# ynalcakan/RGBX_Semantic_Segmentation

Measured on AMD Instinct MI355X. Metric: train images/sec CMX-B2 480x640 bs=2/GPU at 1/2/4/8 MI355X; % MFMA roofline, higher is better.
Workload: dtype bf16

## Files before the change

rgbx_semantic_segmentation_amd/csrc/gemm.hip:

```cpp
#include "gemm_kernels.h"
#include <string.h>
#include <stdlib.h>

using namespace gemmk;
namespace gp = gemmplan;
extern CMX_GEMM_FAST_INST(bf16)
extern CMX_GEMM_FAST_INST(f16)
extern CMX_GEMM_GENERIC_INST(float)
extern CMX_GEMM_GENERIC_INST(bf16)
extern CMX_GEMM_GENERIC_INST(f16)
static_assert(gp::FAST_BK == FBK && gp::GENERIC_BK == BK, "gemm_plan.h counts k-tiles of the kernels' depth");

namespace {
gp::GemmKnobs gemm_knobs() {
  gp::GemmKnobs k;
  k.tiles = cmx_knob("GEMM_TILES", k.tiles);
  k.smallk = cmx_knob("GEMM_SMALLK", k.smallk);
  k.t128 = cmx_knob("GEMM_T128", k.t128);
  k.splitkw = cmx_knob("GEMM_SPLITKW", k.splitkw);
  k.kw = cmx_knob("GEMM_KW", k.kw);
  k.mid = cmx_knob("GEMM_MID", k.mid);
  k.stream = cmx_knob("GEMM_STREAM", k.stream);
  k.stream_k = cmx_knob("GEMM_STREAM_K", k.stream_k);
  k.stream_bpc = cmx_knob("GEMM_STREAM_BPC", k.stream_bpc);
  k.grouped_kt = cmx_knob("GROUPED_KT", k.grouped_kt);
  return k;
}

int launch_gemm(const gp::GemmLaunch& L, const GemmArgs& a, int tA, int tB, int dtype, hipStream_t s) {
  bool ok = true;
  if (L.path == gp::PATH_STREAM) {
    if (dtype == 2) launch_stream<f16>(L, a, tB, s);
    else launch_stream<bf16>(L, a, tB, s);
  } else if (L.path == gp::PATH_TILE) ok = dtype == 2 ? launch_tile<f16>(L, a, tA, tB, s) : launch_tile<bf16>(L, a, tA, tB, s);
  else if (dtype == 1) ok = launch_generic<bf16>(L, a, tA, tB, s);
  else if (dtype == 2) ok = launch_generic<f16>(L, a, tA, tB, s);
  else ok = launch_generic<float>(L, a, tA, tB, s);
  CMX_REQUIRE(ok, CMX_ERR_LAUNCH, "gemm: no kernel for path %d, tile %d x %d, NS %d, KW %d", L.path, L.bm, L.bn, L.ns,
              L.kw);
  if (L.nsplit > 1) {
    if (dtype == 1) launch_reduce<bf16>(L, a, s);
    else if (dtype == 2) launch_reduce<f16>(L, a, s);
    else launch_reduce<float>(L, a, s);
  }
  return CMX_OK;
}

void set_plan(GemmArgs& a, const gp::GemmLaunch& L) {
  a.kt_per_split = L.kt_per_split; a.nsplit = L.nsplit; a.tiles_m = L.tiles_m; a.tiles_n = L.tiles_n;
}

struct RedRec {
  const float* src; float* dst; float* dst2;
  long sg, sb, dg, dg2;
  int ldd, ldd2, G, nblk, rows, cols, csplit, accumulate, zl, cpg, blk0, pad;
};

__global__ __launch_bounds__(256) void reduce_grouped_kernel(const RedRec* __restrict__ recs, int nrec) {
  __shared__ float red[256];
  const int b = blockIdx.x;
  int lo = 0, hi = nrec - 1;
  while (lo < hi) {
    const int mid = (lo + hi + 1) >> 1;
    if (recs[mid].blk0 <= b) lo = mid; else hi = mid - 1;
  }
  const RedRec& r = recs[lo];
  const int zl = r.zl, opb = 256 / zl;
  const int local = b - r.blk0;
  const int g = local / r.cpg, ch = local % r.cpg;
  const int o = threadIdx.x % opb, sl = threadIdx.x / opb;
  const long W = (long)r.rows * r.cols;
  const long w = (long)ch * opb + o;
  float s0 = 0.f, s1 = 0.f, s2 = 0.f, s3 = 0.f;
  if (w < W) {
    const float* p = r.src + (long)g * r.sg + w;
    const long sb = r.sb;
    int k = sl;
    for (; k + 3 * zl < r.nblk; k += 4 * zl) {
      s0 += p[(long)k * sb];
      s1 += p[(long)(k + zl) * sb];
      s2 += p[(long)(k + 2 * zl) * sb];
      s3 += p[(long)(k + 3 * zl) * sb];
    }
    for (; k < r.nblk; k += zl) s0 += p[(long)k * sb];
  }
  float v = (s0 + s1) + (s2 + s3);
// ... 114 lines not shown
              "bias-gradient / upsample / scatter", gh);
  a.gh = gh; a.sAh = p.sAh; a.sBh = p.sBh; a.sCh = p.sCh;
  if (nup) {
    CMX_REQUIRE(up->n <= 3 && G == 1 && !ones_col && N % 8 == 0 && (long)up->oH * up->oW > 0 &&
                M % (up->oH * up->oW) == 0, CMX_ERR_ARG, "gemm: upsample-add epilogue needs G = 1, N %% 8 == 0 and "
                "M a whole number of %d x %d grids", up->oH, up->oW);
    for (int q = 0; q < up->n; ++q) {
      CMX_REQUIRE(up->src[q] && ((uintptr_t)up->src[q] & 15) == 0 && up->h[q] > 0 && up->w[q] > 0, CMX_ERR_ARG,
                  "gemm: upsample-add source %d", q);
      a.up[q] = up->src[q]; a.uh[q] = up->h[q]; a.uw[q] = up->w[q];
    }
    a.nup = up->n; a.uoH = up->oH; a.uoW = up->oW;
  }
  if (p.scR > 0) {
    CMX_REQUIRE(G == 1 || p.sC > 0, CMX_ERR_ARG, "gemm: scatter");
    CMX_REQUIRE((!p.R || lnb) && out_mode == 0 && !ones_col && N == p.scR * p.scR * p.scC && M % (p.scHo * p.scWo) == 0,
                CMX_ERR_ARG, "gemm: patch scatter needs a plain store of N = R*R*C columns");
    a.scatter = 1; a.scH = p.scH; a.scW = p.scW; a.scC = p.scC; a.scR = p.scR; a.scHo = p.scHo; a.scWo = p.scWo;
  }
  set_plan(a, L);
  if (tail) {
    CMX_REQUIRE(fast && N <= 128 && N % 8 == 0 && splitk == 1 && !transA && !transB && out_mode == 0 && !ones_col &&
                    !a.nup && !a.scatter && gh == 1 && !p.mask && a.cvec && dtype != 0,
                CMX_ERR_ARG, "gemm_ln: the LayerNorm epilogue needs the 16-bit path without split-K, forward layouts, a "
                "plain aligned store and N <= 128, N %% 8 == 0 (G=%d M=%d N=%d K=%d)", G, M, N, K);
    CMX_REQUIRE(tail->gamma && tail->beta && tail->y && tail->mean && tail->rstd && ((uintptr_t)tail->y & 15) == 0 &&
                    tail->y != p.C, CMX_ERR_ARG, "gemm_ln: LayerNorm buffers");
    a.tail = 2; a.ln_gamma = tail->gamma; a.ln_beta = tail->beta; a.ln_sg = tail->sg; a.ln_y = tail->y;
    a.ln_mean = tail->mean; a.ln_rstd = tail->rstd; a.ln_eps = tail->eps;
  }
  if (lnb) {
    const bool al = ((uintptr_t)p.C & 15) == 0 && ((uintptr_t)lnb->x & 15) == 0 && ((uintptr_t)p.R & 15) == 0 &&
                    ((uintptr_t)lnb->dy2 & 15) == 0 && ((uintptr_t)lnb->dxs & 15) == 0;
    const bool rows_ok = a.scatter ? (p.scC == 64 || p.scC == 128) && p.scH == p.scHo * p.scR && p.scW == p.scWo * p.scR
                                   : N <= 128 && N % 8 == 0;
    CMX_REQUIRE(fast && splitk == 1 && !transA && transB && out_mode == 0 && !ones_col && !p.bias && p.act == 0 &&
                    !p.mask && !a.nup && gh == 1 && !p.A2 && a.cvec && al && rows_ok && dtype != 0 &&
                    !tail && lnb->x && lnb->gamma && lnb->mean && lnb->rstd && lnb->part && (!lnb->dxs || p.rscale),
                CMX_ERR_ARG, "gemm_ln_bwd: needs the 16-bit dgrad path (transB) without split-K, 16-B aligned rows, "
                "N <= 128 (N %% 8 == 0), no bias / activation (G=%d M=%d N=%d K=%d)", G, M, N, K);
    a.tail = 3; a.ln_gamma = lnb->gamma; a.ln_sg = lnb->sg; a.ln_mean = const_cast<float*>(lnb->mean); a.ln_rstd = const_cast<float*>(lnb->rstd);
    a.lnb_x = lnb->x; a.lnb_dy2 = lnb->dy2; a.lnb_dxs = lnb->dxs; a.lnb_part = lnb->part;
  }
  if (p.plan) {
    const int nblk = gp::multi_blocks(shape, L);
    if (!nblk) return 0;
    a.kt_per_split = (int)gp::cdiv(K, FBK);
    memset(p.plan, 0, sizeof(*p.plan));
    p.plan->a = a; p.plan->tA = transA; p.plan->tB = transB; p.plan->dtype = dtype;
    p.plan->nblk = nblk;
    p.plan->nk64 = a.kt_per_split;
    return nblk;
  }
  const int st = launch_gemm(L, a, transA, transB, dtype, s);
  return st != CMX_OK ? st : cmx_check_launch("gemm");
}
}

extern "C" {

int cmx_gemm(const void* A, const void* A2, const void* B, void* C, const float* bias, const void* R,
             const float* rscale, const void* mask, float* dbias, float* workspace, int G, int M, int N, int K, int K1,
             int64_t lda, int64_t lda2, int64_t ldb, int64_t ldc, int64_t sA, int64_t sA2, int64_t sB, int64_t sC,
             int64_t sbias, int64_t sdb, int rows_per_sample, int transA, int transB, int act, int out_mode,
             int ones_col, int splitk, int dtype, hipStream_t s) {
  GemmProblem p;
  p.A = A; p.A2 = A2; p.B = B; p.C = C; p.bias = bias; p.R = R; p.rscale = rscale; p.mask = mask; p.dbias = dbias;
  p.workspace = workspace; p.G = G; p.M = M; p.N = N; p.K = K; p.K1 = K1; p.lda = lda; p.lda2 = lda2; p.ldb = ldb;
  p.ldc = ldc; p.sA = sA; p.sA2 = sA2; p.sB = sB; p.sC = sC; p.sbias = sbias; p.sdb = sdb;
  p.rows_per_sample = rows_per_sample; p.transA = transA; p.transB = transB; p.act = act; p.out_mode = out_mode;
  p.ones_col = ones_col; p.splitk = splitk; p.dtype = dtype;
  return gemm_impl(p, s);
}

int cmx_gemm_ln(const void* A, const void* A2, const void* B, void* C, const float* bias, const void* R,
                const float* rscale, int G, int M, int N, int K, int K1, int64_t lda, int64_t lda2, int64_t ldb,
                int64_t ldc, int64_t sA, int64_t sA2, int64_t sB, int64_t sC, int64_t sbias, int rows_per_sample,
                int act, const float* ln_gamma, const float* ln_beta, int64_t ln_sg, float ln_eps, void* ln_y,
                float* ln_mean, float* ln_rstd, int dtype, hipStream_t s) {
  const LnTail t{ln_gamma, ln_beta, (long)ln_sg, ln_y, ln_mean, ln_rstd, ln_eps};
  GemmProblem p;
  p.A = A; p.A2 = A2; p.B = B; p.C = C; p.bias = bias; p.R = R; p.rscale = rscale;
  p.G = G; p.M = M; p.N = N; p.K = K; p.K1 = K1; p.lda = lda; p.lda2 = lda2; p.ldb = ldb; p.ldc = ldc;
  p.sA = sA; p.sA2 = sA2; p.sB = sB; p.sC = sC; p.sbias = sbias; p.rows_per_sample = rows_per_sample; p.act = act;
  p.splitk = 1; p.dtype = dtype; p.tail = &t;
  return gemm_impl(p, s);
}

int cmx_gemm_ln_bwd(const void* A, const void* B, void* dx, int G, int M, int N, int K, int64_t lda, int64_t ldb,
                    int64_t ldc, int64_t sA, int64_t sB, int64_t sC, const void* x, const float* gamma, int64_t sg,
                    const float* mean, const float* rstd, const void* dres, const void* dy2, const float* sscale,
                    int rows_per_sample, void* dxs, float* partials, int dtype, hipStream_t s) {
  const LnBwd l{x, gamma, (long)sg, mean, rstd, dy2, dxs, partials};
  GemmProblem p;
  p.A = A; p.B = B; p.C = dx; p.R = dres; p.rscale = sscale; p.G = G; p.M = M; p.N = N; p.K = K;
  p.lda = lda; p.ldb = ldb; p.ldc = ldc; p.sA = sA; p.sB = sB; p.sC = sC; p.rows_per_sample = rows_per_sample;
  p.transB = 1; p.splitk = 1; p.dtype = dtype; p.lnb = &l;
  return gemm_impl(p, s);
}


size_t cmx_gemm_ln_bwd_partials(int G, int M, int N) { return (size_t)G * ((M + 63) / 64) * 2 * N * sizeof(float); }

int cmx_conv_patch_dgrad_ln_bwd(const void* dy, const void* Wt, void* dx, int G, int NIg, int H, int Wd, int C, int R,
                                int Ho, int Wo, int N, int64_t sdy, int64_t sW, int64_t sdx, const void* x,
                                const float* gamma, int64_t sg, const float* mean, const float* rstd, const void* dres,
                                const void* dy2, const float* sscale, int rows_per_sample, void* dxs, float* partials,
// ... 153 lines not shown
                                   int splitk, int blk0) {
  const int M = NIg * Ho * Wo;
  CMX_REQUIRE(rec && G > 0 && N > 0 && C % 8 == 0 && N % 8 == 0 && M % 8 == 0 && tap >= 0 && tap < KH * KW,
              CMX_ERR_SHAPE, "gemm_group_pack_conv_wgrad: bad problem");
  CMX_REQUIRE(((uintptr_t)dy & 15) == 0 && ((uintptr_t)x & 15) == 0 && sdy % 8 == 0 && sx % 8 == 0, CMX_ERR_ARG,
              "gemm_group_pack_conv_wgrad: alignment");
  CMX_REQUIRE((long)NIg * H * Wd * C < (1L << 30) && (long)M * N < (1L << 30), CMX_ERR_SHAPE,
              "gemm_group_pack_conv_wgrad: too large for 31-bit offsets");
  const int ones = dbias ? 1 : 0;
  const int Nk = C + ones;
  const gp::GemmLaunch L = gp::plan_grouped(G, N, C, M, splitk, gemm_knobs());
  CMX_REQUIRE((splitk > 0 ? splitk : L.nsplit) == 1 || workspace, CMX_ERR_ARG,
              "gemm_group_pack_conv_wgrad: split-K needs a workspace");
  GroupRec r{};
  GemmArgs& a = r.a;
  a.A = dy; a.B = x; a.C = dW + (long)tap * C; a.dbias = dbias; a.ws = workspace;
  a.G = G; a.M = N; a.N = Nk; a.K = M; a.K1 = M; a.rows_per_sample = 1;
  a.out_mode = 1; a.ones_col = ones; a.vec = 1;
  a.lda = N; a.sA = sdy; a.ldb = 0; a.sB = sx; a.ldc = (long)KH * KW * C; a.sC = sdW; a.sdb = sdb;
  a.cvec = (((uintptr_t)a.C % 16) == 0) && (a.ldc * 4) % 16 == 0 && (sdW * 4) % 16 == 0;
  a.conv = 2; a.cH = H; a.cW = Wd; a.cC = C; a.cKW = KW; a.cst = stride; a.cpad = pad; a.cHo = Ho; a.cWo = Wo;
  a.ctap = tap;
  set_plan(a, L);
  r.bm = L.bm; r.bn = L.bn;
  r.blk0 = blk0;
  r.nblk = (int)L.grid_x;
  memcpy(rec, &r, sizeof(r));
  return r.nblk;
}

int cmx_conv_implicit_fwd(const void* x, const void* Wt, void* y, const float* bias, float* workspace, int G, int NIg,
                          int H, int Wd, int C, int KH, int KW, int stride, int pad, int Ho, int Wo, int N, int64_t sx,
                          int64_t sW, int64_t sy, int64_t sbias, int splitk, int dtype, hipStream_t s) {
  CMX_REQUIRE((dtype == 1 || dtype == 2) && C % 64 == 0 && N % 8 == 0 && G > 0 && NIg > 0, CMX_ERR_SHAPE,
              "conv_implicit_fwd: bf16 / fp16 with C %% 64 == 0 only (C=%d, N=%d)", C, N);
  CMX_REQUIRE(((uintptr_t)x & 15) == 0 && ((uintptr_t)Wt & 15) == 0 && ((uintptr_t)y & 15) == 0 && sx % 8 == 0 &&
              sW % 8 == 0 && sy % 8 == 0, CMX_ERR_ARG, "conv_implicit_fwd: alignment");
  const long M = (long)NIg * Ho * Wo, K = (long)KH * KW * C;
  CMX_REQUIRE((long)NIg * H * Wd * C < (1L << 30) && M * N < (1L << 31) && (long)N * K < (1L << 30), CMX_ERR_SHAPE,
              "conv_implicit_fwd: too large for 31-bit offsets");
  GemmArgs a{};
  a.A = x; a.B = Wt; a.C = y; a.bias = bias;
  a.G = G; a.M = (int)M; a.N = N; a.K = (int)K; a.K1 = (int)K; a.rows_per_sample = 1; a.vec = 1;
  a.lda = 0; a.sA = sx; a.ldb = K; a.sB = sW; a.ldc = N; a.sC = sy; a.sbias = sbias;
  a.cvec = (N * 2) % 16 == 0 && (sy * 2) % 16 == 0;
  a.conv = 1; a.cH = H; a.cW = Wd; a.cC = C; a.cKW = KW; a.cst = stride; a.cpad = pad; a.cHo = Ho; a.cWo = Wo;
  gp::GemmShape shape;
  shape.G = G; shape.M = (int)M; shape.N = N; shape.K = (int)K; shape.dtype = dtype; shape.fast = 1;
  shape.splitk = splitk; shape.tile_only = 1;
  const gp::GemmLaunch L = gp::plan_gemm(shape, gemm_knobs(), cu_count());
  CMX_REQUIRE((splitk > 0 ? splitk : L.nsplit) == 1 || workspace, CMX_ERR_ARG, "conv_implicit_fwd: split-K needs a workspace");
  a.ws = workspace;
  set_plan(a, L);
  const int st = launch_gemm(L, a, 0, 0, dtype, s);
  return st != CMX_OK ? st : cmx_check_launch("conv_implicit_fwd");
}

int cmx_gemm_grouped(const void* recs, int nrec, int total_blocks, int dtype, hipStream_t s) {
  CMX_REQUIRE(dtype == 1 || dtype == 2, CMX_ERR_DTYPE, "gemm_grouped: operands bf16 (1) or fp16 (2), got %d", dtype);
  CMX_REQUIRE(recs && nrec > 0 && total_blocks > 0, CMX_ERR_ARG, "gemm_grouped: empty launch");
  return cmx_gemm_grouped_capped(recs, nrec, total_blocks, 0, dtype, s);
}

int cmx_gemm_grouped_capped(const void* recs, int nrec, int total_blocks, int max_blocks, int dtype, hipStream_t s) {
  CMX_REQUIRE(dtype == 1 || dtype == 2, CMX_ERR_DTYPE, "gemm_grouped: operands bf16 (1) or fp16 (2), got %d", dtype);
  CMX_REQUIRE(recs && nrec > 0 && total_blocks > 0, CMX_ERR_ARG, "gemm_grouped: empty launch");
  CMX_REQUIRE(max_blocks <= 0 || max_blocks % 8 == 0, CMX_ERR_ARG, "gemm_grouped: max_blocks %d not a multiple of 8",
              max_blocks);
  static int& chunk = cmx_knob("GROUPED_CHUNK", 64);
  const GroupRec* rr = (const GroupRec*)recs;
  const int grid = max_blocks > 0 && max_blocks < total_blocks ? max_blocks : total_blocks;
  if (grid < total_blocks) {
    if (dtype == 2)
      hipLaunchKernelGGL((gemm_grouped_kernel<f16, 2, true>), dim3(grid), dim3(256), 0, s, rr, nrec, chunk, total_blocks);
    else
      hipLaunchKernelGGL((gemm_grouped_kernel<bf16, 2, true>), dim3(grid), dim3(256), 0, s, rr, nrec, chunk, total_blocks);
  } else if (dtype == 2) {
    hipLaunchKernelGGL((gemm_grouped_kernel<f16>), dim3(grid), dim3(256), 0, s, rr, nrec, chunk, total_blocks);
  } else {
    hipLaunchKernelGGL((gemm_grouped_kernel<bf16>), dim3(grid), dim3(256), 0, s, rr, nrec, chunk, total_blocks);
  }
  return cmx_check_launch("gemm_grouped");
}

size_t cmx_reduce_record_size(void) { return sizeof(RedRec); }

int cmx_reduce_pack(void* rec, const float* src, float* dst, float* dst2, int G, int nblk, int64_t sg, int64_t sb,
                    int rows, int cols, int csplit, int64_t dg, int ldd, int64_t dg2, int ldd2, int accumulate,
                    int blk0) {
  CMX_REQUIRE(rec && src && dst && G > 0 && nblk > 0 && rows > 0 && cols > 0 && blk0 >= 0, CMX_ERR_SHAPE,
              "reduce_pack: bad reduction");
  CMX_REQUIRE(csplit >= cols || (dst2 && csplit >= 0), CMX_ERR_ARG, "reduce_pack: columns past csplit need dst2");
  RedRec r{};
  r.src = src; r.dst = dst; r.dst2 = dst2; r.sg = sg; r.sb = sb; r.dg = dg; r.dg2 = dg2;
  r.ldd = ldd; r.ldd2 = ldd2; r.G = G; r.nblk = nblk; r.rows = rows; r.cols = cols; r.csplit = csplit;
  r.accumulate = accumulate;
  r.zl = nblk <= 8 ? 1 : (nblk <= 64 ? 4 : 16);
  r.cpg = (int)cdiv((long)rows * cols, 256 / r.zl);
  r.blk0 = blk0;
  memcpy(rec, &r, sizeof(r));
  return r.cpg * G;
}

int cmx_reduce_grouped(const void* recs, int nrec, int total_blocks, hipStream_t s) {
  CMX_REQUIRE(recs && nrec > 0 && total_blocks > 0, CMX_ERR_ARG, "reduce_grouped: empty launch");
  hipLaunchKernelGGL(reduce_grouped_kernel, dim3(total_blocks), dim3(256), 0, s, (const RedRec*)recs, nrec);
  return cmx_check_launch("reduce_grouped");
// ... 4 lines not shown
```

rgbx_semantic_segmentation_amd/csrc/gemm_kernels.h:

```cpp
#pragma once
#include "cmx_mfma.h"
#include "cmx_dma.h"
#include "gemm_plan.h"
#include <string.h>
#include <stdlib.h>

namespace gemmk {
using gemmplan::GemmLaunch;

struct GemmArgs {
  const void* A; const void* A2; const void* B; void* C; const float* bias; const void* R; const float* rscale;
  float* dbias; float* ws;
  int G, M, N, K, K1, kt_per_split, rows_per_sample, act, out_mode, tiles_m, tiles_n, ones_col, nsplit, vec, cvec;
  long lda, lda2, ldb, ldc, sA, sA2, sB, sC, sbias, sdb;
  int conv, cH, cW, cC, cKW, cst, cpad, cHo, cWo, ctap;
  const void* up[3];
  int uh[3], uw[3], nup, uoH, uoW;
  int scatter, scH, scW, scC, scR, scHo, scWo;
  int gh;
  long sAh, sBh, sCh;
  const void* mask;
  int tail;
  float ln_eps;
  const float* ln_gamma;
// ... 62 lines not shown
    if constexpr (sizeof(T) == 4) {
      load_vec<T>(u + t.r00 * ld + 4, a + 4);
      load_vec<T>(u + t.r01 * ld + 4, b + 4);
      load_vec<T>(u + t.r10 * ld + 4, c + 4);
      load_vec<T>(u + t.r11 * ld + 4, d + 4);
    }
#pragma unroll
    for (int e = 0; e < 8; ++e) v[e] += t.w00 * a[e] + t.w01 * b[e] + t.w10 * c[e] + t.w11 * d[e];
  }
}

__device__ __forceinline__ long goff(const GemmArgs& p, int g, long s, long sh) {
  return p.gh > 1 ? (long)(g / p.gh) * s + (long)(g % p.gh) * sh : (long)g * s;
}

__device__ __forceinline__ long scatter_offset(const GemmArgs& p, int g, int i, int j) {
  const int hw = p.scHo * p.scWo;
  const int n = i / hw, r = i - n * hw, oy = r / p.scWo, ox = r - oy * p.scWo;
  const int tap = j / p.scC, c = j - tap * p.scC, kh = tap / p.scR, kw = tap - kh * p.scR;
  return (long)g * p.sC + (((long)n * p.scH + oy * p.scR + kh) * p.scW + ox * p.scR + kw) * p.scC + c;
}

template <bool EXT = true>
__device__ __forceinline__ long c_offset(const GemmArgs& p, int g, int i, int j) {
  if constexpr (EXT) {
    if (p.scatter) return scatter_offset(p, g, i, j);
  }
  return goff(p, g, p.sC, p.sCh) + (long)i * p.ldc + j;
}

template <typename T, bool EXT = false>
__device__ __forceinline__ void epi_store(const GemmArgs& p, int g, int i, int j, float acc) {
  const float bj = p.bias ? p.bias[(long)g * p.sbias + j] : 0.f;
  if constexpr (EXT) {
    if (p.nup) acc += up_add1<T>(p, i, j);
  }
  float v = act_fwd(acc + bj, p.act);
  const long off = c_offset<EXT>(p, g, i, j);
  if (p.R) {
    const float sc = p.rscale ? p.rscale[((long)g * p.M + i) / p.rows_per_sample] : 1.f;
    v = to_f32(reinterpret_cast<const T*>(p.R)[off]) + sc * v;
  }
  if (p.mask && !(to_f32(reinterpret_cast<const T*>(p.mask)[off]) > 0.f)) v = 0.f;
  if (p.out_mode == 0) reinterpret_cast<T*>(p.C)[off] = from_f32<T>(v);
  else if (p.out_mode == 1) reinterpret_cast<float*>(p.C)[off] = v;
  else reinterpret_cast<float*>(p.C)[off] += v;
}

__device__ __forceinline__ void dbias_store(const GemmArgs& p, int g, int i, float v) {
  float* d = p.dbias + (long)g * p.sdb + i;
  *d = p.out_mode == 2 ? *d + v : v;
}

template <typename T>
__device__ __forceinline__ void epi_store8(const GemmArgs& p, int g, int i, int j, int nv, float* v) {
  if (nv < 8 || !p.cvec) {
    for (int e = 0; e < nv; ++e) epi_store<T, true>(p, g, i, j + e, v[e]);
    return;
  }
  if (p.bias) {
    const float* bp = p.bias + (long)g * p.sbias + j;
#pragma unroll
    for (int e = 0; e < 8; ++e) v[e] += bp[e];
  }
  if (p.nup) up_add8<T>(p, i, j, v);
  if (p.act) {
#pragma unroll
    for (int e = 0; e < 8; ++e) v[e] = act_fwd(v[e], p.act);
  }
  const long off = c_offset(p, g, i, j);
  if (p.R) {
    const float sc = p.rscale ? p.rscale[((long)g * p.M + i) / p.rows_per_sample] : 1.f;
    float rv[8];
    load_vec<T>(reinterpret_cast<const T*>(p.R) + off, rv);
    if constexpr (sizeof(T) == 4) load_vec<T>(reinterpret_cast<const T*>(p.R) + off + 4, rv + 4);
#pragma unroll
    for (int e = 0; e < 8; ++e) v[e] = rv[e] + sc * v[e];
  }
  if (p.mask) {
    float mv[8];
    load_vec<T>(reinterpret_cast<const T*>(p.mask) + off, mv);
    if constexpr (sizeof(T) == 4) load_vec<T>(reinterpret_cast<const T*>(p.mask) + off + 4, mv + 4);
#pragma unroll
    for (int e = 0; e < 8; ++e) v[e] = mv[e] > 0.f ? v[e] : 0.f;
  }
  if (p.out_mode == 0) {
    store_vec<T>(reinterpret_cast<T*>(p.C) + off, v);
    if constexpr (sizeof(T) == 4) store_vec<T>(reinterpret_cast<T*>(p.C) + off + 4, v + 4);
  } else {
    float4* d = reinterpret_cast<float4*>(reinterpret_cast<float*>(p.C) + off);
    if (p.out_mode == 2) {
      const float4 o0 = d[0], o1 = d[1];
      v[0] += o0.x; v[1] += o0.y; v[2] += o0.z; v[3] += o0.w; v[4] += o1.x; v[5] += o1.y; v[6] += o1.z; v[7] += o1.w;
    }
    d[0] = make_float4(v[0], v[1], v[2], v[3]);
    d[1] = make_float4(v[4], v[5], v[6], v[7]);
  }
}

__device__ __forceinline__ float* slab(const GemmArgs& p, int g, int z) {
  const int Nr = p.ones_col ? p.N - 1 : p.N;
  return p.ws + (((long)g * p.nsplit + z) * p.M) * Nr;
}
__device__ __forceinline__ float* slab_db(const GemmArgs& p, int G, int g, int z) {
  const int Nr = p.N - 1;
  return p.ws + (long)G * p.nsplit * p.M * Nr + ((long)g * p.nsplit + z) * p.M;
}

constexpr int FBK = 64;
template <int ROWS>
__device__ __forceinline__ int tr_swz(int kk) {
  if constexpr (ROWS == 128) return ((kk & 3) << 2) | ((kk >> 2) & 3);
  else return ((kk >> 1) & 1) << 2;
}

template <int ROWS>
__device__ __forceinline__ void stage_k(const i32x4 rsrc, char* img, long ld, int row0, int nrows, int k0, int kend,
                                        int w, int lane) {
  constexpr int NI = ROWS / 32;
#pragma unroll
  for (int n = 0; n < NI; ++n) {
    const int row = (w * NI + n) * 8 + (lane >> 3);
    const int c = (lane & 7) ^ ((row >> 1) & 7);
// ... 458 lines not shown
  };
  auto img = [](float* cs, int il, int c4) { return cs + il * 64 + ((c4 ^ (il & 15)) << 2); };
  auto epilogue = [&](int q, float* cs) {
    int g, tm, tn;
    tile_of(q, g, tm, tn);
    const int i0 = tm * 64, j0 = tn * 64;
    const int r = lane & 31, h = lane >> 5;
#pragma unroll
    for (int g4 = 0; g4 < 4; ++g4) {
      const int il = wm * 32 + r, c4 = wn * 8 + 2 * g4 + h;
      *reinterpret_cast<float4*>(img(cs, il, c4)) =
          make_float4(acc[4 * g4], acc[4 * g4 + 1], acc[4 * g4 + 2], acc[4 * g4 + 3]);
    }
    __syncthreads();
    constexpr int TPR = 8, RPP = 256 / TPR;
    const int jl = (threadIdx.x % TPR) * 8, j = j0 + jl;
    const bool live = j < nreal;
    const int nv = min(8, nreal - j);
#pragma unroll
    for (int pass = 0; pass < 64 / RPP; ++pass) {
      const int il = pass * RPP + threadIdx.x / TPR;
      const int i = i0 + il;
      if (i >= p.M) break;
      const float4 u0 = *reinterpret_cast<const float4*>(img(cs, il, jl / 4));
      const float4 u1 = *reinterpret_cast<const float4*>(img(cs, il, jl / 4 + 1));
      float v[8] = {u0.x, u0.y, u0.z, u0.w, u1.x, u1.y, u1.z, u1.w};
      if constexpr (EPI == 2) {
        if (live) epi_store8<E>(p, g, i, j, 8, v);
        row_layernorm<E, TPR>(p, g, i, j, jl, live, v);
      } else {
        if (live) epi_store8<E>(p, g, i, j, nv, v);
      }
    }
  };
  stage(0, smem);
  vm_wait<0>();
  __syncthreads();
  int cur = 0;
  for (int st = 0; st < S; ++st) {
    if (st + 1 < S) stage(st + 1, smem + (cur ^ 1) * STREAM_SLOT);
    compute(smem + cur * STREAM_SLOT);
    const int q = st / nk;
    if (st - q * nk == nk - 1) {
      __syncthreads();
      epilogue(q, reinterpret_cast<float*>(smem + cur * STREAM_SLOT));
      acc = zero16();
    }
    vm_wait<0>();
    __syncthreads();
    cur ^= 1;
  }
}

constexpr int MULTI_MAX = 4;
struct GemmMulti {
  GemmArgs a[MULTI_MAX];
  int blk0[MULTI_MAX + 1];
  int n;
};

template <int NS, int KW, bool TB, typename E>
__global__ __launch_bounds__(256 * KW, (NS == 2 && KW == 1) ? 5 : 2) void gemm_multi_kernel(const GemmMulti m) {
  __shared__ __attribute__((aligned(1024))) char smem[gemm_smem_bytes<64, 64, NS, KW>()];
  const int b = blockIdx.x;
  int i = 0;
#pragma unroll
  for (int j = 1; j < MULTI_MAX; ++j)
    if (j < m.n && b >= m.blk0[j]) i = j;
  const int nb = m.blk0[i + 1] - m.blk0[i];
  gemm_bf16_body<64, 64, false, TB, NS, KW, E>(m.a[i], xcd_tile(b - m.blk0[i], nb), smem);
}

struct GroupRec {
  GemmArgs a;
  int bm, bn, blk0, nblk;
};

__device__ __forceinline__ int xcd_chunk_tile(int b, int nt, int ch) {
  const int full = nt / (8 * ch) * (8 * ch);
  if (b >= full) return b;
  const int x = b & 7, j = b >> 3;
  return ((j / ch) * 8 + x) * ch + j % ch;
}

template <typename E, int NS>
__device__ __forceinline__ void grouped_tile(const GroupRec* __restrict__ recs, int nrec, int lin, char* smem) {
  int lo = 0, hi = nrec - 1;
  while (lo < hi) {
    const int mid = (lo + hi + 1) >> 1;
    if (recs[mid].blk0 <= lin) lo = mid; else hi = mid - 1;
  }
  const GroupRec& r = recs[lo];
  const GemmArgs p = r.a;
  const int local = lin - r.blk0;
  if (r.bm == 128 && r.bn == 128) gemm_bf16_body<128, 128, true, true, NS, 1, E>(p, local, smem);
  else if (r.bm == 128) gemm_bf16_body<128, 64, true, true, NS, 1, E>(p, local, smem);
  else if (r.bn == 128) gemm_bf16_body<64, 128, true, true, NS, 1, E>(p, local, smem);
  else gemm_bf16_body<64, 64, true, true, NS, 1, E>(p, local, smem);
}

template <typename E, int NS = 2, bool LOOP = false>
__global__ __launch_bounds__(256, 2) void gemm_grouped_kernel(const GroupRec* __restrict__ recs, int nrec,
                                                                             int chunk, int total) {
  __shared__ __attribute__((aligned(1024))) char smem[gemm_smem_bytes<128, 128, NS>()];
  if constexpr (!LOOP) {
    const int b = blockIdx.x;
// ... 238 lines not shown
void launch_reduce(const GemmLaunch& L, const GemmArgs& a, hipStream_t s) {
  const dim3 grid(L.red_grid_x, L.red_grid_y);
  if (L.red_zl == 16) hipLaunchKernelGGL((splitk_reduce_kernel<T, 16>), grid, dim3(256), 0, s, a);
  else if (L.red_zl == 4) hipLaunchKernelGGL((splitk_reduce_kernel<T, 4>), grid, dim3(256), 0, s, a);
  else hipLaunchKernelGGL((splitk_reduce_kernel<T, 1>), grid, dim3(256), 0, s, a);
}

template <int BM, int BN, int NS, int KW, typename E>
void launch_tile_as(const GemmArgs& a, dim3 grid, int tA, int tB, hipStream_t s) {
  if constexpr (BM == 64 && (BN == 64 || (BN == 128 && KW == 1))) {
    if (a.tail == 2) {
      hipLaunchKernelGGL((gemm_bf16_kernel<64, BN, false, false, NS, KW, E, 2>), grid, dim3(256 * KW), 0, s, a);
      return;
    }
    if (a.tail == 3) {
      hipLaunchKernelGGL((gemm_bf16_kernel<64, BN, false, true, NS, KW, E, 3>), grid, dim3(256 * KW), 0, s, a);
      return;
    }
  }
#define CMX_GEMM_LAUNCH(TA, TB) hipLaunchKernelGGL((gemm_bf16_kernel<BM, BN, TA, TB, NS, KW, E>), grid, dim3(256 * KW), 0, s, a)
  if (!tA && !tB) CMX_GEMM_LAUNCH(false, false);
  else if (!tA && tB) CMX_GEMM_LAUNCH(false, true);
  else if (tA && tB) CMX_GEMM_LAUNCH(true, true);
  else CMX_GEMM_LAUNCH(true, false);
#undef CMX_GEMM_LAUNCH
}

template <typename E>
bool launch_tile(const GemmLaunch& L, const GemmArgs& a, int tA, int tB, hipStream_t s) {
#define CMX_GEMM_TILE(BM, BN, NS, KW)                                   \
  if (L.bm == BM && L.bn == BN && L.ns == NS && L.kw == KW) {           \
    launch_tile_as<BM, BN, NS, KW, E>(a, dim3(L.grid_x), tA, tB, s);    \
    return true;                                                        \
  }
  CMX_GEMM_TILE(64, 64, 2, 4) CMX_GEMM_TILE(64, 64, 4, 2) CMX_GEMM_TILE(64, 64, 2, 2)
  CMX_GEMM_TILE(64, 64, 4, 1) CMX_GEMM_TILE(64, 64, 2, 1) CMX_GEMM_TILE(64, 128, 4, 1) CMX_GEMM_TILE(64, 128, 2, 1)
  CMX_GEMM_TILE(128, 64, 4, 1) CMX_GEMM_TILE(128, 64, 2, 1) CMX_GEMM_TILE(128, 128, 4, 1) CMX_GEMM_TILE(128, 128, 2, 1)
#undef CMX_GEMM_TILE
  return false;
}

inline int cu_count() {
  static const int n = [] {
    int dev = 0, c = 0;
    if (hipGetDevice(&dev) != hipSuccess || hipDeviceGetAttribute(&c, hipDeviceAttributeMultiprocessorCount, dev) !=
                                               hipSuccess)
      c = 0;
    return c > 0 ? c : 256;
  }();
  return n;
}

template <typename E>
void launch_stream(const GemmLaunch& L, const GemmArgs& a, int tB, hipStream_t s) {
  const dim3 grid(L.grid_x);
  if (a.tail == 2) hipLaunchKernelGGL((gemm_stream_kernel<false, E, 2>), grid, dim3(256), 0, s, a);
  else if (tB) hipLaunchKernelGGL((gemm_stream_kernel<true, E, 0>), grid, dim3(256), 0, s, a);
  else hipLaunchKernelGGL((gemm_stream_kernel<false, E, 0>), grid, dim3(256), 0, s, a);
}

template <typename T>
bool launch_generic(const GemmLaunch& L, const GemmArgs& a, int tA, int tB, hipStream_t s) {
  const dim3 grid(L.grid_x, L.grid_y, L.grid_z);
  const bool ext = a.nup || a.scatter;
#define CMX_GEMM_GENERIC(BM, BN, TA, TB, EXT)                                                             \
  if (L.bm == BM && L.bn == BN && !tA == !TA && !tB == !TB && ext == EXT) {                               \
    hipLaunchKernelGGL((gemm_generic_kernel<T, BM, BN, TA, TB, EXT>), grid, dim3(256), 0, s, a);          \
    return true;                                                                                          \
  }
#define CMX_GEMM_GENERIC_TILE(BM, BN)                                                                      \
  CMX_GEMM_GENERIC(BM, BN, false, false, false) CMX_GEMM_GENERIC(BM, BN, false, true, false)              \
  CMX_GEMM_GENERIC(BM, BN, true, true, false) CMX_GEMM_GENERIC(BM, BN, true, false, false)                \
  CMX_GEMM_GENERIC(BM, BN, false, false, true) CMX_GEMM_GENERIC(BM, BN, false, true, true)                \
  CMX_GEMM_GENERIC(BM, BN, true, true, true) CMX_GEMM_GENERIC(BM, BN, true, false, true)
  CMX_GEMM_GENERIC_TILE(64, 64) CMX_GEMM_GENERIC_TILE(64, 128) CMX_GEMM_GENERIC_TILE(128, 64) CMX_GEMM_GENERIC_TILE(128, 128)
#undef CMX_GEMM_GENERIC_TILE
#undef CMX_GEMM_GENERIC
  return false;
}

inline bool fast_ok(const void* A, const void* A2, const void* B, int M, int N, int K, int K1, long lda, long lda2, long ldb,
             long sA, long sA2, long sB, int tA, int tB, int ones_col) {
  const int nb = ones_col ? N - 1 : N;
  auto al = [](const void* p) { return ((uintptr_t)p & 15) == 0; };
  if (!al(A) || !al(B) || (A2 && !al(A2))) return false;
  if (lda % 8 || ldb % 8 || sA % 8 || sB % 8 || (K % 8 && !(tA && tB))) return false;
  if (tA ? M % 8 : false) return false;
  if (tB ? nb % 8 : false) return false;
  if (A2 && (K1 % FBK || lda2 % 8 || sA2 % 8 || tA)) return false;
  const long extA = tA ? (long)K * lda : (long)M * lda;
  const long extB = tB ? (long)K * ldb : (long)nb * ldb;
  const long extA2 = A2 ? (long)M * lda2 : 0;
  const long lim = (1L << 30) - 64;
  return extA < lim && extB < lim && extA2 < lim;
}

}

#define CMX_GEMM_GENERIC_INST(T) \
  template bool gemmk::launch_generic<T>(const gemmk::GemmLaunch&, const gemmk::GemmArgs&, int, int, hipStream_t);
#define CMX_GEMM_FAST_INST(E) \
  template bool gemmk::launch_tile<E>(const gemmk::GemmLaunch&, const gemmk::GemmArgs&, int, int, hipStream_t);
```

rgbx_semantic_segmentation_amd/csrc/gemm_plan.h:

```cpp
#pragma once
#include <stdint.h>

#ifndef CMX_STREAM_LB
#define CMX_STREAM_LB 4
#endif

namespace gemmplan {

constexpr int FAST_BK = 64, GENERIC_BK = 32;

inline long cdiv(long a, long b) { return (a + b - 1) / b; }

struct GemmKnobs {
  int tiles = 1;
  int smallk = 256;
  int t128 = 400;
  int splitkw = 1;
  int kw = 2;
  int mid = 50;
  int stream = 1024;
  int stream_k = 128;
  int stream_bpc = CMX_STREAM_LB;
  int grouped_kt = 48;
};
// ... 78 lines not shown
  L.ns = L.kw == 4 || blocks > 256 ? 2 : 4;
  if (L.kw > 1) L.kt_per_split = split_k(nk64, L.kw).kt;
  L.grid_x = (unsigned)blocks; L.grid_y = L.grid_z = 1;
  L.block = 256u * L.kw;
}

inline GemmLaunch plan_gemm(const GemmShape& p, const GemmKnobs& k, int num_cu) {
  GemmLaunch L{};
  const int nb = p.ones_col ? p.N - 1 : p.N;
  const int split = p.splitk > 0 ? p.splitk
                    : p.fast     ? auto_split(p.G, p.M, p.N, p.K, p.ones_col, k)
                                 : generic_split(p.G, p.M, p.N, p.K);
  const int nk = (int)cdiv(p.K, p.fast ? FAST_BK : GENERIC_BK);
  const KSplit ks = split_k(nk, split);
  L.kt_per_split = ks.kt; L.nsplit = ks.n;
  L.kw = 1; L.block = 256;
  if (!p.fast) {
    L.path = PATH_GENERIC;
    L.bm = tile_dim(p.M); L.bn = tile_dim(p.N);
    L.tiles_m = (int)cdiv(p.M, L.bm); L.tiles_n = (int)cdiv(p.N, L.bn);
    L.grid_x = (unsigned)(L.tiles_m * L.tiles_n); L.grid_y = (unsigned)p.G; L.grid_z = (unsigned)L.nsplit;
  } else {
    plan_tiles(p.G, p.M, nb, p.K, k, &L.bm, &L.bn);
    if (p.row_ln || p.ln_bwd) L.bm = 64, L.bn = p.N <= 64 ? 64 : 128;
    if (p.ln_bwd && p.scC) L.bn = p.scC;
    const bool plain64 = L.bm == 64 && L.bn == 64 && L.nsplit == 1 && !p.tile_only && !p.ln_bwd && !p.scC && !p.nup;
    if (k.mid > 0 && plain64 && !p.row_ln && nb >= 128) {
      const long t64 = cdiv(p.M, 64) * cdiv(nb, 64) * p.G, slots = 5L * num_cu;
      if (t64 > slots && t64 * 100 <= slots * (100 + k.mid)) L.bn = 128;
    }
    L.tiles_m = (int)cdiv(p.M, L.bm); L.tiles_n = (int)cdiv(nb, L.bn);
    const long tiles = (long)L.tiles_m * L.tiles_n * p.G;
    if (k.stream > 0 && tiles >= k.stream && p.K <= k.stream_k && plain64 && L.bn == 64 && !p.transA && !p.a2 &&
        !p.ones_col && p.gh == 1 && (!p.row_ln || p.N <= 64)) {
      L.path = PATH_STREAM;
      const int bpc = k.stream_bpc > 0 && k.stream_bpc <= CMX_STREAM_LB ? k.stream_bpc : CMX_STREAM_LB;
      long grid = (long)bpc * num_cu;
      if (grid > tiles) grid = tiles;
      L.grid_x = (unsigned)((grid + 7) / 8 * 8); L.grid_y = L.grid_z = 1;
    } else {
      L.path = PATH_TILE;
      tile_waves(L, tiles * L.nsplit, (int)cdiv(p.K, FAST_BK), k.kw,
                 L.bm == 64 && L.bn == 64 && L.nsplit == 1 && !p.ones_col);
    }
  }
  if (L.nsplit > 1) {
    const long work = (long)p.M * cdiv(nb, 8) + (p.ones_col ? p.M : 0);
    L.red_zl = L.nsplit >= 32 ? 16 : L.nsplit >= 8 ? 4 : 1;
    L.red_grid_x = (unsigned)cdiv(work, 256 / L.red_zl); L.red_grid_y = (unsigned)p.G;
  }
  return L;
}

inline int multi_blocks(const GemmShape& p, const GemmLaunch& L) {
  if (!p.fast || L.nsplit != 1 || p.ones_col || p.nup || p.scC || p.gh != 1 || p.transA) return 0;
  return L.bm == 64 && L.bn == 64 ? L.tiles_m * L.tiles_n * p.G : 0;
}

inline GemmLaunch plan_multi(int total_blocks, int min_nk64, const GemmKnobs& k) {
  GemmLaunch L{};
  L.path = PATH_TILE; L.bm = L.bn = 64; L.nsplit = 1; L.kt_per_split = min_nk64;
  tile_waves(L, total_blocks, min_nk64, k.kw < 2 ? k.kw : 2, true);
  return L;
}

inline GemmLaunch plan_grouped(int G, int M, int nb, int K, int splitk, const GemmKnobs& k) {
  GemmLaunch L{};
  const KSplit ks = split_k((int)cdiv(K, FAST_BK), splitk > 0 ? splitk : grouped_split(K, k));
  L.path = PATH_TILE; L.kt_per_split = ks.kt; L.nsplit = ks.n;
  L.bm = tile_dim(M); L.bn = tile_dim(nb);
  L.tiles_m = (int)cdiv(M, L.bm); L.tiles_n = (int)cdiv(nb, L.bn);
  L.grid_x = (unsigned)(L.tiles_m * L.tiles_n * G * L.nsplit);
  return L;
}

}
```

rgbx_semantic_segmentation_amd/roofline.py:

```python
from __future__ import annotations

import glob
import json
import os

import torch

from . import deferred, _lib
from .floor import step_work

PEAK_BF16_TFLOPS = 2516.6
PEAK_HBM_GBS = 8000.0
_ROOT = os.path.dirname(os.path.dirname(os.path.abspath(__file__)))


RIDGE_FLOP_PER_BYTE = PEAK_BF16_TFLOPS * 1e12 / (PEAK_HBM_GBS * 1e9)


def _pmc_traffic(kernel: str, workload: str, blocks: int):
    for path in sorted(glob.glob(os.path.join(_ROOT, "profiles", "*pmc*.json")), reverse=True):
        try:
            d = json.load(open(path))
        except (OSError, ValueError):
            continue
        if d.get("workload") != workload:
            continue
        k = d.get("kernels", {}).get(kernel)
        if k and k.get("hbm_bytes_per_launch") and k.get("blocks") in (None, blocks):
            return k["hbm_bytes_per_launch"], os.path.relpath(path, _ROOT)
    return None, None


GEMM_FAMILY = ("cmx_gemm", "cmx_gemm_ln", "cmx_gemm_multi", "cmx_conv_implicit_fwd", "cmx_decoder_fuse_fwd",
               "cmx_conv_patch_dgrad", "cmx_gemm_ln_bwd", "cmx_conv_patch_dgrad_ln_bwd")


def _family_traffic(kernels, workload: str):
    for path in sorted(glob.glob(os.path.join(_ROOT, "profiles", "*pmc*.json")), reverse=True):
        try:
            d = json.load(open(path))
        except (OSError, ValueError):
            continue
        if d.get("workload") != workload:
            continue
        ks = [d.get("kernels", {}).get(k) for k in kernels]
        ks = [k for k in ks if k and k.get("hbm_bytes_per_launch") and k.get("launches")]
        if ks:
            n = sum(k["launches"] for k in ks)
            return sum(k["hbm_bytes_per_launch"] * k["launches"] for k in ks) / n, os.path.relpath(path, _ROOT)
    return None, None


FAMILY_RE = (
    ("wgrad", r"gemm_grouped_kernel|reduce_grouped_kernel"),
    ("gemm", r"gemm_bf16_kernel|gemm_stream|gemm_multi|gemm_generic|splitk_reduce"),
    ("sra", r"sra_"),
    ("dwconv", r"dw2_|dw_"),
    ("layernorm", r"ln_fwd|ln_bwd|rowln"),
    ("adamw", r"adamw"),
    ("batchnorm", r"bn_"),
    ("frm", r"pool_|linear_fwd|linear_bwd|combine_|frm_|reduce_partials"),
    ("ffm", r"ffm_"),
    ("ce", r"ce_|upsample|loss_cells|loss_finalize"),
    ("bilinear", r"bilinear|adj3_|up3_"),
    ("im2col", r"im2col|col2im"),
    ("pe1", r"pe1_"),
)


def family_of(kernel: str) -> str:
    import re
    for fam, rx in FAMILY_RE:
        if re.search(rx, kernel):
            return fam
    return "other"


def trace_kernels(run_step, steps: int):
    from torch.profiler import profile, ProfilerActivity
    torch.cuda.synchronize()
    with profile(activities=[ProfilerActivity.CUDA]) as prof:
        for _ in range(steps):
            run_step()
        torch.cuda.synchronize()
    out = []
    for e in prof.profiler.kineto_results.events():
        if e.device_type() != torch.autograd.DeviceType.CUDA:
            continue
        name = e.name()
        if "Memcpy" in name or "Memset" in name:
            continue
        out.append((name, e.start_ns() / 1e3, e.duration_ns() / 1e3))
    out.sort(key=lambda r: r[1])
    return out


STEP_FIRST = "step_masks_kernel"


def split_steps(recs):
    idx = [i for i, r in enumerate(recs) if STEP_FIRST in r[0]]
    if not idx:
        return []
    segs = [recs[a:b] for a, b in zip(idx, idx[1:] + [len(recs)])]
    full = max(len(sg) for sg in segs)
    return [sg for sg in segs if len(sg) == full]


# ... 189 lines not shown
```

Baseline: 292.1.

## Add panel GEMM kernel keeping B fragments in registers for small-K streaming GEMMs

Adds a new gemm_panel_kernel for the streaming path when K is at most two k-tiles and N is a multiple of 64. Each block loads its B column panel into registers once, then walks many 32-row A strips through a shared-memory ring with counted vmem waits, staging the output through an LDS transpose. The bias is also held in LDS. The intent is to stop reloading B and to overlap A loads with MFMA and epilogue work for these skinny GEMMs. The cost is added register pressure, a fixed grid-to-work mapping, and a specialised epilogue that skips the nup and extended offset features.

Result: no change. 294.2, median of 6 (+0.7%).

```diff
diff --git a/rgbx_semantic_segmentation_amd/csrc/gemm.hip b/rgbx_semantic_segmentation_amd/csrc/gemm.hip
--- a/rgbx_semantic_segmentation_amd/csrc/gemm.hip
+++ b/rgbx_semantic_segmentation_amd/csrc/gemm.hip
@@ -27,11 +27,13 @@
   return k;
 }
 
-int launch_gemm(const gp::GemmLaunch& L, const GemmArgs& a, int tA, int tB, int dtype, hipStream_t s) {
+int launch_gemm(const gp::GemmLaunch& L, const gp::GemmShape& shape, const GemmArgs& a, int tA, int tB, int dtype,
+                hipStream_t s) {
   bool ok = true;
   if (L.path == gp::PATH_STREAM) {
-    if (dtype == 2) launch_stream<f16>(L, a, tB, s);
-    else launch_stream<bf16>(L, a, tB, s);
+    const bool panel = cmx_knob("GEMM_PANEL", 1) != 0 && gp::stream_panel_ok(shape, L);
+    if (dtype == 2) launch_stream<f16>(L, a, tB, panel, s);
+    else launch_stream<bf16>(L, a, tB, panel, s);
   } else if (L.path == gp::PATH_TILE) ok = dtype == 2 ? launch_tile<f16>(L, a, tA, tB, s) : launch_tile<bf16>(L, a, tA, tB, s);
   else if (dtype == 1) ok = launch_generic<bf16>(L, a, tA, tB, s);
   else if (dtype == 2) ok = launch_generic<f16>(L, a, tA, tB, s);
@@ -252,7 +254,7 @@
     p.plan->nk64 = a.kt_per_split;
     return nblk;
   }
-  const int st = launch_gemm(L, a, transA, transB, dtype, s);
+  const int st = launch_gemm(L, shape, a, transA, transB, dtype, s);
   return st != CMX_OK ? st : cmx_check_launch("gemm");
 }
 }
@@ -512,7 +514,7 @@
   CMX_REQUIRE((splitk > 0 ? splitk : L.nsplit) == 1 || workspace, CMX_ERR_ARG, "conv_implicit_fwd: split-K needs a workspace");
   a.ws = workspace;
   set_plan(a, L);
-  const int st = launch_gemm(L, a, 0, 0, dtype, s);
+  const int st = launch_gemm(L, shape, a, 0, 0, dtype, s);
   return st != CMX_OK ? st : cmx_check_launch("conv_implicit_fwd");
 }
 
diff --git a/rgbx_semantic_segmentation_amd/csrc/gemm_kernels.h b/rgbx_semantic_segmentation_amd/csrc/gemm_kernels.h
--- a/rgbx_semantic_segmentation_amd/csrc/gemm_kernels.h
+++ b/rgbx_semantic_segmentation_amd/csrc/gemm_kernels.h
@@ -138,23 +138,27 @@
   *d = p.out_mode == 2 ? *d + v : v;
 }
 
-template <typename T>
+template <typename T, bool BIAS = true, bool EXT = true>
 __device__ __forceinline__ void epi_store8(const GemmArgs& p, int g, int i, int j, int nv, float* v) {
-  if (nv < 8 || !p.cvec) {
-    for (int e = 0; e < nv; ++e) epi_store<T, true>(p, g, i, j + e, v[e]);
-    return;
-  }
-  if (p.bias) {
+  if constexpr (BIAS) {
+    if (nv < 8 || !p.cvec) {
+      for (int e = 0; e < nv; ++e) epi_store<T, EXT>(p, g, i, j + e, v[e]);
+      return;
+    }
+  }
+  if (BIAS && p.bias) {
     const float* bp = p.bias + (long)g * p.sbias + j;
 #pragma unroll
     for (int e = 0; e < 8; ++e) v[e] += bp[e];
   }
-  if (p.nup) up_add8<T>(p, i, j, v);
+  if constexpr (EXT) {
+    if (p.nup) up_add8<T>(p, i, j, v);
+  }
   if (p.act) {
 #pragma unroll
     for (int e = 0; e < 8; ++e) v[e] = act_fwd(v[e], p.act);
   }
-  const long off = c_offset(p, g, i, j);
+  const long off = c_offset<EXT>(p, g, i, j);
   if (p.R) {
     const float sc = p.rscale ? p.rscale[((long)g * p.M + i) / p.rows_per_sample] : 1.f;
     float rv[8];
@@ -719,6 +723,133 @@
   }
 }
 
+constexpr int PANEL_RING = 16384, PANEL_IMG = 4096, PANEL_SMEM = PANEL_RING + 4 * PANEL_IMG + 1024;
+
+__device__ __forceinline__ void lgkm_wait0() { __builtin_amdgcn_s_waitcnt(0xC07F); }
+
+__device__ __forceinline__ void vm_wait_n(int n) {
+  switch (n) {
+    case 0: vm_wait<0>(); break;
+    case 1: vm_wait<1>(); break;
+    case 2: vm_wait<2>(); break;
+    case 3: vm_wait<3>(); break;
+    case 4: vm_wait<4>(); break;
+    case 5: vm_wait<5>(); break;
+    case 6: vm_wait<6>(); break;
+    case 7: vm_wait<7>(); break;
+    case 8: vm_wait<8>(); break;
+    case 9: vm_wait<9>(); break;
+    case 10: vm_wait<10>(); break;
+    case 11: vm_wait<11>(); break;
+    case 12: vm_wait<12>(); break;
+    case 13: vm_wait<13>(); break;
+    default: vm_wait<14>(); break;
+  }
+}
+
+template <bool TB, typename E, int NK>
+__global__ __launch_bounds__(256, NK == 1 ? 4 : 3) void gemm_panel_kernel(const GemmArgs p) {
+  constexpr int SLOT = NK * 4096, NSLOT = PANEL_RING / SLOT;
+  constexpr int ST_PER_EPI = 4;
+  __shared__ __attribute__((aligned(1024))) char smem[PANEL_SMEM];
+  const int lane = threadIdx.x & 63, w = threadIdx.x >> 6;
+  const int ncg = p.tiles_n >> 2, pairs = p.G * ncg;
+  const int nbx = gridDim.x >> 3, xb = blockIdx.x & 7, bi = blockIdx.x >> 3;
+  const int th = (p.M + 31) >> 5;
+  const int per = (th + 7) >> 3, lo = xb * per, hi = min(th, lo + per);
+  if (lo >= hi) return;
+  const int avail = NK == 1 ? nbx / pairs : max(1, nbx * 3 / 4 / pairs);
+  const int walk = (hi - lo + avail - 1) / avail, nslots = (hi - lo + walk - 1) / walk;
+  const int slot = bi / pairs, pair = bi - slot * pairs;
+  if (slot >= nslots) return;
+  const int g = pair / ncg, cg = pair - g * ncg;
+  const int first = lo + slot;
+  const int nu = (hi - first + nslots - 1) / nslots;
+  const i32x4 rA = make_rsrc(reinterpret_cast<const E*>(p.A) + goff(p, g, p.sA, p.sAh));
+  const i32x4 rB = make_rsrc(reinterpret_cast<const E*>(p.B) + goff(p, g, p.sB, p.sBh));
+  const int j0 = (4 * cg + w) * 64;
+
+  frag8<E> fb[NK][FBK / 16][2];
+  char* wb = smem + w * 8192;
+#pragma unroll
+  for (int kt = 0; kt < NK; ++kt) {
+#pragma unroll
+    for (int wq = 0; wq < 4; ++wq) {
+      if constexpr (TB) stage_r<64>(rB, wb, p.ldb, j0, p.N, kt * FBK, p.K, wq, lane);
+      else stage_k<64>(rB, wb, p.ldb, j0, p.N, kt * FBK, p.K, wq, lane);
+    }
+    vm_wait<0>();
+    __syncthreads();
+#pragma unroll
+    for (int s = 0; s < FBK / 16; ++s)
+#pragma unroll
+      for (int b = 0; b < 2; ++b) {
+        if constexpr (TB) fb[kt][s][b] = frag_r<E, 64>(wb, b * 32, s, lane);
+        else fb[kt][s][b] = frag_k<E>(wb, b * 32, s, lane);
+      }
+    lgkm_wait0();
+  }
+  float* bs = reinterpret_cast<float*>(smem + PANEL_RING + 4 * PANEL_IMG);
+  {
+    bs[threadIdx.x] = p.bias ? p.bias[(long)g * p.sbias + cg * 256 + threadIdx.x] : 0.f;
+  }
+  __syncthreads();
+
+  auto stage = [&](int q, char* buf) {
+    const int i0 = (first + q * nslots) * 32;
+#pragma unroll
+    for (int kt = 0; kt < NK; ++kt) stage_k<32>(rA, buf + kt * 4096, p.lda, i0, p.M, kt * FBK, p.K, w, lane);
+  };
+  const int pro = min(NSLOT, nu);
+#pragma unroll
+  for (int q = 0; q < NSLOT; ++q)
+    if (q < pro) stage(q, smem + q * SLOT);
+
+  float* cs = reinterpret_cast<float*>(smem + PANEL_RING + w * PANEL_IMG);
+  const int r = lane & 31, h = lane >> 5, jc = lane & 3;
+  int cur = 0;
+  for (int u = 0; u < nu; ++u) {
+    const int last = u == 0 ? pro - 1 : min(nu - 1, u - 2 + NSLOT);
+    vm_wait_n((last - u) * NK + ST_PER_EPI * min(u, NSLOT - 1));
+    __syncthreads();
+    if (u >= 1 && u - 1 + NSLOT < nu) stage(u - 1 + NSLOT, smem + (cur == 0 ? NSLOT - 1 : cur - 1) * SLOT);
+    const char* ab = smem + cur * SLOT;
+    const int i0 = (first + u * nslots) * 32;
+#pragma unroll
+    for (int b = 0; b < 2; ++b) {
+      f32x16 acc = zero16();
+#pragma unroll
+      for (int kt = 0; kt < NK; ++kt)
+#pragma unroll
+        for (int s = 0; s < FBK / 16; ++s) acc = MF<E>::mma(fb[kt][s][b], frag_k<E>(ab + kt * 4096, 0, s, lane), acc);
+#pragma unroll
+      for (int g4 = 0; g4 < 4; ++g4)
+        *reinterpret_cast<float4*>(cs + r * 32 + (((2 * g4 + h) ^ (r & 7)) << 2)) =
+            make_float4(acc[4 * g4], acc[4 * g4 + 1], acc[4 * g4 + 2], acc[4 * g4 + 3]);
+      const int jl = b * 32 + jc * 8, j = j0 + jl;
+#pragma unroll 1
+      for (int pass = 0; pass < 2; ++pass) {
+        const int il = pass * 16 + (lane >> 2), i = i0 + il;
+        const float4 u0 = *reinterpret_cast<const float4*>(cs + il * 32 + (((2 * jc) ^ (il & 7)) << 2));
+        const float4 u1 = *reinterpret_cast<const float4*>(cs + il * 32 + (((2 * jc + 1) ^ (il & 7)) << 2));
+        float v[8] = {u0.x, u0.y, u0.z, u0.w, u1.x, u1.y, u1.z, u1.w};
+        if (i >= p.M) continue;
+        if (p.cvec) {
+          if (p.bias) {
+            const float4 b0 = *reinterpret_cast<const float4*>(bs + w * 64 + jl);
+            const float4 b1 = *reinterpret_cast<const float4*>(bs + w * 64 + jl + 4);
+            v[0] += b0.x; v[1] += b0.y; v[2] += b0.z; v[3] += b0.w; v[4] += b1.x; v[5] += b1.y; v[6] += b1.z; v[7] += b1.w;
+          }
+          epi_store8<E, false, false>(p, g, i, j, 8, v);
+        } else {
+          epi_store8<E, true, false>(p, g, i, j, 8, v);
+        }
+      }
+    }
+    cur = cur + 1 == NSLOT ? 0 : cur + 1;
+  }
+}
+
 constexpr int MULTI_MAX = 4;
 struct GemmMulti {
   GemmArgs a[MULTI_MAX];
@@ -1063,8 +1194,18 @@
 }
 
 template <typename E>
-void launch_stream(const GemmLaunch& L, const GemmArgs& a, int tB, hipStream_t s) {
+void launch_stream(const GemmLaunch& L, const GemmArgs& a, int tB, bool panel, hipStream_t s) {
   const dim3 grid(L.grid_x);
+  if (panel) {
+    if (a.K <= FBK) {
+      if (tB) hipLaunchKernelGGL((gemm_panel_kernel<true, E, 1>), grid, dim3(256), 0, s, a);
+      else hipLaunchKernelGGL((gemm_panel_kernel<false, E, 1>), grid, dim3(256), 0, s, a);
+    } else {
+      if (tB) hipLaunchKernelGGL((gemm_panel_kernel<true, E, 2>), grid, dim3(256), 0, s, a);
+      else hipLaunchKernelGGL((gemm_panel_kernel<false, E, 2>), grid, dim3(256), 0, s, a);
+    }
+    return;
+  }
   if (a.tail == 2) hipLaunchKernelGGL((gemm_stream_kernel<false, E, 2>), grid, dim3(256), 0, s, a);
   else if (tB) hipLaunchKernelGGL((gemm_stream_kernel<true, E, 0>), grid, dim3(256), 0, s, a);
   else hipLaunchKernelGGL((gemm_stream_kernel<false, E, 0>), grid, dim3(256), 0, s, a);
diff --git a/rgbx_semantic_segmentation_amd/csrc/gemm_plan.h b/rgbx_semantic_segmentation_amd/csrc/gemm_plan.h
--- a/rgbx_semantic_segmentation_amd/csrc/gemm_plan.h
+++ b/rgbx_semantic_segmentation_amd/csrc/gemm_plan.h
@@ -154,6 +154,12 @@
   return L;
 }
 
+inline bool stream_panel_ok(const GemmShape& p, const GemmLaunch& L) {
+  if (L.path != PATH_STREAM || p.row_ln || p.ln_bwd) return false;
+  if (p.N % 64 || L.tiles_n % 4 || p.K > 2 * FAST_BK) return false;
+  return (long)p.G * (L.tiles_n / 4) <= (long)(L.grid_x / 8);
+}
+
 inline int multi_blocks(const GemmShape& p, const GemmLaunch& L) {
   if (!p.fast || L.nsplit != 1 || p.ones_col || p.nup || p.scC || p.gh != 1 || p.transA) return 0;
   return L.bm == 64 && L.bn == 64 ? L.tiles_m * L.tiles_n * p.G : 0;
diff --git a/rgbx_semantic_segmentation_amd/roofline.py b/rgbx_semantic_segmentation_amd/roofline.py
--- a/rgbx_semantic_segmentation_amd/roofline.py
+++ b/rgbx_semantic_segmentation_amd/roofline.py
@@ -53,7 +53,7 @@
 
 FAMILY_RE = (
     ("wgrad", r"gemm_grouped_kernel|reduce_grouped_kernel"),
-    ("gemm", r"gemm_bf16_kernel|gemm_stream|gemm_multi|gemm_generic|splitk_reduce"),
+    ("gemm", r"gemm_bf16_kernel|gemm_stream|gemm_panel|gemm_multi|gemm_generic|splitk_reduce"),
     ("sra", r"sra_"),
     ("dwconv", r"dw2_|dw_"),
     ("layernorm", r"ln_fwd|ln_bwd|rowln"),
```
